# gooey-audio/libgooey

Hardware: NVIDIA B200
Metric: voice-samples/sec (higher is better)
Workload: dtype f32

## Files before the change

libgooey_b200/csrc/kernels.cuh:

```cuda
#pragma once
#include <cuda_runtime.h>
#include "voices2.cuh"
#include "../../include/gooey_batch.h"

namespace gd {

constexpr int TILE = 32;

template <class S> __device__ __forceinline__ void load_words(S& s, const uint32_t* base, int slot, int n_pad, int w0) {
  constexpr int W = sizeof(S) / 4;
  uint32_t* w = reinterpret_cast<uint32_t*>(&s);
#pragma unroll
  for (int i = 0; i < W; i++) w[i] = base[(size_t)(w0 + i) * n_pad + slot];
}
template <class S> __device__ __forceinline__ void store_words(const S& s, uint32_t* base, int slot, int n_pad, int w0) {
  constexpr int W = sizeof(S) / 4;
  const uint32_t* w = reinterpret_cast<const uint32_t*>(&s);
#pragma unroll
  for (int i = 0; i < W; i++) base[(size_t)(w0 + i) * n_pad + slot] = w[i];
}

struct KickV {
  using State = KickState; using Ctl = KickCtl; using Aud = KickAud; using Span = KickSpan;
  static constexpr bool FAST = true; static constexpr int NPL = KICK_PLANES; static constexpr uint32_t ID = GOOEY_INSTRUMENT_KICK;
  struct Run { KickDer d; int j_act; };
  static __device__ __forceinline__ float tick(State& s, const double* tt, const RateCtx& rc) { return kick_tick(s, tt, rc); }
  static __device__ __forceinline__ void slow_event(State& s, const VoiceEvent& e, const double* tt, const RateCtx&) {
    uint32_t r = 0; kick_event(s.c, e, tt, r); kick_span_begin(s.a, s.c, r);
  }
  static __device__ __forceinline__ bool settled(const Ctl& c) { return params_settled<K_NP>(c.cur, c.tgt); }
  static __device__ __forceinline__ void event(Ctl& c, const VoiceEvent& e, const double* tt, uint32_t& r) { kick_event(c, e, tt, r); }
  static __device__ __forceinline__ void plan(Ctl& c, uint32_t r, const double* tt, int ja, int jb, Span& sp) { kick_plan(c, r, tt, ja, jb, sp); }
  static __device__ __forceinline__ int front_end(const Span& sp) { return sp.j_act; }
  static __device__ __forceinline__ void front(const Span& sp, double now, uint32_t, float sr, float* o) {
// ... 108 lines not shown
  const VoiceEvent* events;
  const uint32_t* ev_begin;
  const double* tt;
  int frames;
  float* out; long long stride;
  RateCtx rc;
  uint8_t* mode;
  void* spans;
  const uint32_t* span_off;
  uint32_t* n_spans;
  uint32_t* span_cursor;
  float* planes;
  long long plane_stride;
  int pitch;
  int chunk0, chunk_frames;
  const ModRoute* routes; const uint32_t* route_begin;
  const float* mod_planes; long long mod_pitch; int mod_frame0;
};

__device__ __forceinline__ void store_tile_voice_major(const float* tile , float* out, long long stride, int row0,
                                                        const uint32_t* rows, uint32_t row_mask, int f0, int nf, int lane) {
  const bool vec_ok = (nf == TILE) && ((stride & 3) == 0) && ((f0 & 3) == 0) && ((reinterpret_cast<uintptr_t>(out) & 15) == 0);
  if (vec_ok) {
    const int c = (lane & 7) * 4;
#pragma unroll
    for (int k = 0; k < 8; k++) {
      const int r = k * 4 + (lane >> 3);
      if ((row_mask >> r) & 1u) {
        const float* src = tile + r * 33 + c;
        float4 v = make_float4(src[0], src[1], src[2], src[3]);
// ... 6 lines not shown
      if (!((row_mask >> r) & 1u)) continue;
      const long long row = rows ? (long long)rows[r] : (long long)(row0 + r);
      if (lane < nf) out[row * stride + f0 + lane] = tile[r * 33 + lane];
    }
  }
}
__device__ __forceinline__ void load_tile_rows(float* tile , const float* plane, int pitch, int row0, int n_rows, int c0, int lane) {
  const int c = (lane & 7) * 4;
#pragma unroll
  for (int k = 0; k < 8; k++) {
    const int r = k * 4 + (lane >> 3);
    if (r < n_rows) {
      const float4 v = *reinterpret_cast<const float4*>(plane + (size_t)(row0 + r) * pitch + c0 + c);
      float* dst = tile + r * 33 + c;
      dst[0] = v.x; dst[1] = v.y; dst[2] = v.z; dst[3] = v.w;
    }
  }
}

__device__ __forceinline__ void load_tile_rows_any(float* tile , const float* plane, long long pitch, int row0, int n_rows, int c0, int nf, int lane) {
  for (int r = 0; r < n_rows; r++)
    if (lane < nf) tile[r * 33 + lane] = plane[(long long)(row0 + r) * pitch + c0 + lane];
}

template <class V, int BLOCK>
__global__ void __launch_bounds__(BLOCK) slow_kernel(const VoiceLaunch L) {
  __shared__ float tiles[BLOCK / 32][TILE * 33];
  const int v = blockIdx.x * BLOCK + threadIdx.x;
  const int lane = threadIdx.x & 31;
  const int warp = threadIdx.x >> 5;
// ... 177 lines not shown
```

libgooey_b200/csrc/pool.cuh:

```cuda
#pragma once
#include <algorithm>
#include <atomic>
#include <map>
#include <type_traits>
#include <mutex>
#include <tuple>
#include "device_rt.h"
#include "wave.cuh"
#include "coop.cuh"
#include "gran_wave.cuh"
#include "bass_wave.cuh"
#include "poly_wave.cuh"
#include "patch.h"

namespace gh {

extern std::atomic<uint64_t> g_launches;

struct KernelStat { uint64_t launches = 0; double ms = 0.0; double voice_frames = 0.0; };
std::map<std::string, KernelStat>& kernel_stats();
std::mutex& kernel_stats_mutex();
struct KernelTimer {
  struct Rec { cudaEvent_t t0, t1; const char* key; double units; };
  std::vector<Rec> recs;
// ... 134 lines not shown
  }
};
ClockTable& clock_table(float sr);

enum class Back { Wave, Coop, Serial };
constexpr int COOP_FROM = 4096;
constexpr int COOP_NV = 16;
constexpr int SERIAL_FROM = 12288;
inline bool serial_backend() { const char* e = getenv("GOOEY_B200_BACKEND"); return e && strcmp(e, "serial") == 0; }
template <class V> inline Back choose_back(int cnt) {
  if (serial_backend()) return Back::Serial;
  if (std::is_same<V, gd::TomV>::value) return cnt >= COOP_FROM ? Back::Coop : Back::Wave;
  return cnt >= SERIAL_FROM ? Back::Serial : Back::Wave;
}
template <class V> struct WaveOf;
template <> struct WaveOf<gd::KickV> { using W = gd::wave::KickW; static constexpr const char* name = "wave_kernel<KickW>"; };
template <> struct WaveOf<gd::SnareV> { using W = gd::wave::SnareW; static constexpr const char* name = "wave_kernel<SnareW>"; };
template <> struct WaveOf<gd::HatV> { using W = gd::wave::HatW; static constexpr const char* name = "wave_kernel<HatW>"; };
template <> struct WaveOf<gd::TomV> { using W = gd::wave::TomW; static constexpr const char* name = "wave_kernel<TomW>"; };

inline void coop_launch(int cnt, cudaStream_t s, const gd::VoiceLaunch& L) {
  using SM = gd::coop::Smem<gd::coop::TomC, COOP_NV>;
  auto kernel = gd::coop::coop_kernel<gd::coop::TomC, COOP_NV>;
  func_attr_once((const void*)kernel, cudaFuncAttributeMaxDynamicSharedMemorySize, (int)sizeof(SM));
  func_attr_once((const void*)kernel, cudaFuncAttributePreferredSharedMemoryCarveout, (int)cudaSharedmemCarveoutMaxShared);
  kernel<<<(cnt + COOP_NV - 1) / COOP_NV, COOP_NV * 32, sizeof(SM), s>>>(L);
}

template <class K> inline void same_carveout(K kernel) {
  func_attr_once((const void*)kernel, cudaFuncAttributePreferredSharedMemoryCarveout, (int)cudaSharedmemCarveoutMaxShared);
}
#define GH_LAUNCH(kernel, grid, block, stream, ...) do { same_carveout(kernel); kernel<<<grid, block, 0, stream>>>(__VA_ARGS__); } while (0)

template <class V> inline void slow_launch(const gd::VoiceLaunch& L, cudaStream_t s) {
// ... 23 lines not shown
template <> inline const char* launch_back<gd::GranV>(const gd::VoiceLaunch& L, cudaStream_t s) {
  GH_LAUNCH((gd::gran_wave_kernel<4>), (L.n + 3) / 4, 128, s, L);
  return "gran_wave_kernel";
}

constexpr int CHUNK_FRAMES = 8192;
template <class V> struct TypeRunner {
  using State = typename V::State;
  Pool<State> pool;
  std::vector<uint32_t> slots, rows, ev_begin, span_off;
  std::vector<gd::VoiceEvent> ev_flat;
  std::vector<gd::ModRoute> routes_flat; std::vector<uint32_t> route_begin;
  DevBuf<gd::ModRoute> d_routes; DevBuf<uint32_t> d_route_begin;
  const float* mod_planes = nullptr; long long mod_pitch = 0; int mod_frame0 = 0;
  DevBuf<uint32_t> d_slots, d_rows, d_ev_begin, d_span_off, d_n_spans, d_span_cursor;
  DevBuf<gd::VoiceEvent> d_events;
  DevBuf<uint8_t> d_mode, d_spans;
  DevBuf<float> d_planes[2];
  cudaStream_t sB = nullptr, sC = nullptr, sS = nullptr;
  cudaEvent_t evA = nullptr, evB[2] = {nullptr, nullptr}, evC[2] = {nullptr, nullptr}, evDoneC = nullptr, evDoneS = nullptr;
  KernelTimer timer;
  std::vector<cudaEvent_t> evChunk;
  int launched_chunks = 0;
  static int chunk_of(int frames) { return std::min(CHUNK_FRAMES, (frames + 31) & ~31); }
  void wait_chunk(cudaStream_t s, int i) {
    if (n() == 0) return;
    if (launched_chunks == 0) { GH_CUDA(cudaStreamWaitEvent(s, evDoneC, 0)); return; }
    GH_CUDA(cudaStreamWaitEvent(s, evDoneS, 0));
    GH_CUDA(cudaStreamWaitEvent(s, evChunk[std::min(i, launched_chunks - 1)], 0));
  }
// ... 46 lines not shown
    memset(&L, 0, sizeof L);
    L.state = pool.d.p; L.n = cnt; L.n_pad = pool.cap;
    L.slots = d_slots.p; L.rows = d_rows.p; L.row0 = 0;
    L.events = d_events.p; L.ev_begin = d_ev_begin.p; L.tt = tt; L.frames = frames; L.out = out; L.stride = stride; L.rc = rc;
    if (!routes_flat.empty() && mod_planes) {
      d_routes.upload(routes_flat.data(), routes_flat.size(), sC);
      d_route_begin.upload(route_begin.data(), route_begin.size(), sC);
      L.routes = d_routes.p; L.route_begin = d_route_begin.p; L.mod_planes = mod_planes; L.mod_pitch = mod_pitch; L.mod_frame0 = mod_frame0;
    }
    const char* key = nullptr;
    if constexpr (V::FAST) {
      using Span = typename V::Span;
      d_span_off.upload(span_off.data(), span_off.size(), sC);
      d_n_spans.alloc(cnt); d_span_cursor.alloc(cnt); d_mode.alloc(cnt);
      d_spans.alloc((size_t)span_off.back() * sizeof(Span));
      const int chunk = chunk_of(frames);
      const int rows_pad = pad32(cnt);
      const size_t plane_floats = (size_t)rows_pad * chunk;
      d_planes[0].alloc(plane_floats * V::NPL); d_planes[1].alloc(plane_floats * V::NPL);
      L.mode = d_mode.p; L.spans = d_spans.p; L.span_off = d_span_off.p; L.n_spans = d_n_spans.p; L.span_cursor = d_span_cursor.p;
      L.plane_stride = (long long)plane_floats; L.pitch = chunk;
      GH_LAUNCH((gd::plan_kernel<V>), (cnt + 63) / 64, 64, sC, L);
      g_launches.fetch_add(1, std::memory_order_relaxed);
      GH_CUDA(cudaGetLastError());
      GH_CUDA(cudaEventRecord(evA, sC));
      GH_CUDA(cudaStreamWaitEvent(sB, evA, 0));
      GH_CUDA(cudaStreamWaitEvent(sS, evA, 0));
      GH_LAUNCH((gd::slow_kernel<V, 32>), (cnt + 31) / 32, 32, sS, L);
      g_launches.fetch_add(1, std::memory_order_relaxed);
      GH_CUDA(cudaGetLastError());
      GH_CUDA(cudaEventRecord(evDoneS, sS));
      int i = 0;
      for (int c0 = 0; c0 < frames; c0 += chunk, i++) {
        const int b = i & 1;
        L.chunk0 = c0; L.chunk_frames = std::min(chunk, frames - c0);
        L.planes = d_planes[b].p;
        if (i >= 2) GH_CUDA(cudaStreamWaitEvent(sB, evC[b], 0));
        const int bpv = (L.chunk_frames + 255) / 256;
        GH_LAUNCH((gd::front_kernel<V, 256>), (unsigned)((size_t)cnt * bpv), 256, sB, L, bpv);
        GH_CUDA(cudaGetLastError());
        GH_CUDA(cudaEventRecord(evB[b], sB));
        GH_CUDA(cudaStreamWaitEvent(sC, evB[b], 0));
        timer.begin(sC);
        key = launch_back<V>(L, sC);
        GH_CUDA(cudaGetLastError());
        timer.end(sC, key, (double)cnt * L.chunk_frames);
        GH_CUDA(cudaEventRecord(evC[b], sC));
        if ((int)evChunk.size() <= i) { cudaEvent_t e; GH_CUDA(cudaEventCreateWithFlags(&e, cudaEventDisableTiming)); evChunk.push_back(e); }
        GH_CUDA(cudaEventRecord(evChunk[i], sC));
        g_launches.fetch_add(2, std::memory_order_relaxed);
      }
      launched_chunks = i;
    } else {
      timer.begin(sC);
      key = launch_back<V>(L, sC);
// ... 50 lines not shown
```

libgooey_b200/csrc/voices.cuh:

```cuda
#pragma once
#include "dsp.cuh"
#include "events.h"

namespace gd {

struct RateCtx {
  float sr;
  double dt;
  float smooth15;
  float smooth10, smooth30, smooth50;
  float click_alpha;
  float asym_down;
  PinkCoef pink;
};
G_HD RateCtx make_rate_ctx(float sr) {
  RateCtx c;
  c.sr = sr;
  c.dt = 1.0 / (double)sr;
  c.smooth15 = smooth_coeff(sr, 15.0f);
  c.smooth10 = smooth_coeff(sr, 10.0f);
  c.smooth30 = smooth_coeff(sr, 30.0f);
  c.smooth50 = smooth_coeff(sr, 50.0f);
  c.click_alpha = 1.0f - gm::g_expf(-2.0f * PI_F * 8000.0f / sr);
  c.asym_down = 1.0f - gm::g_expf(-1.0f / 100.0f);
// ... 195 lines not shown
  a.click_hp += rc.click_alpha * hp;
  float filt_click = hp * (1.0f + 4.0f * 0.1f);
  float noise_out = 0.0f;
  if (d.noise_amount > 0.001f) {
    float pn = pink_tick(a.pink, rc.pink);
    rlp_set(a.noise_lp, sr, d.noise_cut, d.noise_res);
    float fn = rlp_process(a.noise_lp, pn);
    noise_out = fn * f.ne * d.noise_amount * 0.5f;
  }
  float total = f.p1 + filt_click + noise_out;
  a.ws.drive = d.drive;
  a.ws.feedback = d.feedback;
  fbws_set_cutoff(a.ws, sr, d.fb_cutoff);
  float od = fbws_process(a.ws, total);
  return od * f.amp * d.va * d.volume;
}
G_D float kick_tick(KickState& s, const double* tt, const RateCtx& rc) {
  KickCtl& c = s.c;
  const double now = tt[c.k];
  c.k += 1;
#pragma unroll
  for (int i = 0; i < K_NP; i++) smooth_tick(c.cur[i], c.tgt[i], rc.smooth15);
  if (!c.active) return 0.0f;
  kick_live(c);
  const KickDer d = kick_derive(c);
#ifdef __CUDA_ARCH__
  const KickFront f = d.drive <= 8.0f ? kick_front<true>(c, d, now, rc.sr) : kick_front<false>(c, d, now, rc.sr);
#else
  const KickFront f = kick_front(c, d, now, rc.sr);
#endif
// ... 191 lines not shown
}
G_HD bool snare_still_active(const SnareCtl& c) {
  bool classic = env_active(c.tonal_osc_env) || env_active(c.noise_osc_env) || env_active(c.crack_env);
  bool ds = env_active(c.tonal_env) || env_active(c.main_noise_env) || env_active(c.tail_env) || env_active(c.amp_env) || c.pm.active;
  return classic || ds;
}
G_D float snare_back(SnareAud& a, const SnareDer& d, const SnareFront& f, const RateCtx& rc) {
  chamb_set(a.filt, rc.sr, d.cutoff, d.res);
  float filtered = chamb_process(a.filt, f.raw_noise, d.filter_type);
  float noise_out = filtered * f.cne * d.noise_mix;
  float total = f.tonal_out + noise_out + f.crack_out;
  a.ws.drive = d.drive;
  float od = ws_process(a.ws, total);
  return od * f.amp * d.va * d.volume;
}
G_D float snare_tick(SnareState& s, const double* tt, const RateCtx& rc) {
  SnareCtl& c = s.c;
  const double now = tt[c.k];
  c.k += 1;
  bool changing = false;
#pragma unroll
  for (int i = 0; i < S_NP; i++) { smooth_tick(c.cur[i], c.tgt[i], rc.smooth15); changing |= (c.cur[i] != c.tgt[i]); }
  if (!c.active) return 0.0f;
  if (changing) {
    float cvs = 0.7f + 0.3f * c.velocity;
    c.tonal_vol = clampf(c.cur[S_TONAL], 0.0f, 1.0f);
    c.noise_vol = clampf(c.cur[S_NOISE] * 0.8f, 0.0f, 1.0f);
    c.crack_vol = clampf(c.cur[S_BRIGHTNESS] * 0.4f * cvs, 0.0f, 1.0f);
  }
  snare_live(c);
// ... 135 lines not shown
  else { float n = u64_to_f32(xorshift64s_next(a.white)) / 18446744073709551616.0f; noise = (n * 2.0f) - 1.0f; }
  float mod_out = hat_osc(a.mod_phase, d.pitch_hz * 0.1f, sr, noise * 0.25f);
  float main_out = hat_osc(a.main_phase, d.pitch_hz, sr, mod_out * 0.75f);
  hp_set(a.hp1, sr, d.pitch_hz, 1.0f);
  float filtered = biquad_process(a.hp1, main_out);
  if (d.db24) { hp_set(a.hp2, sr, d.pitch_hz, 1.0f); filtered = biquad_process(a.hp2, filtered) * 0.8f; }
  float env = f.env;
  if (env >= a.env_smooth) a.env_smooth = env; else a.env_smooth += rc.asym_down * (env - a.env_smooth);
  env = a.env_smooth;
  float out = filtered * env * d.vel035 * 0.35f;
  tpt_set(a.svf, sr, d.tone_hz, 0.5f);
  float lo, bd, hi;
  tpt_process(a.svf, out, lo, bd, hi);
  float o = hi * d.volume;
  if (env_complete && a.env_smooth < 1e-4f) a.active = 0;
  return o;
}
G_D float hat_tick(HatState& s, const double* tt, const RateCtx& rc) {
  HatCtl& c = s.c;
  const double now = tt[c.k];
  c.k += 1;
#pragma unroll
  for (int i = 0; i < H_NP; i++) smooth_tick(c.cur[i], c.tgt[i], rc.smooth15);
  if (!s.a.active) return 0.0f;
  hat_live(c);
  const HatDer d = hat_derive(c);
  HatFront f;
  f.env = maxenv_value(c.env, now);
  return hat_back(s.a, d, f, maxenv_complete(c.env), rc);
}
// ... 273 lines not shown
```

libgooey_b200/csrc/wave.cuh:

```cuda
#pragma once
#include "kernels.cuh"

namespace gd { namespace wave {

__device__ __forceinline__ float shup(float v, int d) { return __shfl_up_sync(0xffffffffu, v, d); }
__device__ __forceinline__ float shl(float v, int n) { return __shfl_sync(0xffffffffu, v, n); }
__device__ __forceinline__ bool gall(bool p) { return __all_sync(0xffffffffu, p); }
__device__ __forceinline__ unsigned gballot(bool p) { return __ballot_sync(0xffffffffu, p); }
__device__ __forceinline__ void gsync() { __syncwarp(); }

struct Geo1 { float m[5]; float ap; };
struct Geo2 { float a; float m[5]; float ap; };

__device__ __forceinline__ Geo1 make_geo1(float a, int lane) {
  Geo1 g; float p = a, ap = 1.0f; const int e = lane + 1;
#pragma unroll
  for (int i = 0; i < 5; i++) { g.m[i] = lane >= (1 << i) ? p : 0.0f; if (e & (1 << i)) ap *= p; p *= p; }
  if (e & 32) ap *= p;
  g.ap = ap;
  return g;
}
__device__ __forceinline__ Geo2 make_geo2(float a, int lane) {
  Geo2 g; g.a = a; float p = a * a, ap = 1.0f;
#pragma unroll
// ... 147 lines not shown

__device__ __forceinline__ float w_tanh(float x) {
  const float ax = fabsf(x);
  const float e = __expf(2.0f * ax);
  const float t = 1.0f - __fdividef(2.0f, e + 1.0f);
  return copysignf(t, x);
}
__device__ __forceinline__ float w_gain_comp(FbShaper& w, float env) {
  const float reference = fmaxf(env, 0.05f);
  const float driven = fmaxf(fabsf(w_tanh(reference * w.drive)), 1e-6f);
  const float comp_no_fb = w_tanh(reference) / driven;
  const float makeup = fbws_makeup(w);
  const float taming = 1.0f / (1.0f + comp_no_fb * w.feedback * 0.25f);
  return fminf(comp_no_fb * taming * makeup, 3.0f);
}
__device__ __forceinline__ float wrap01(float x) { return x < 1.0f ? x : (x < 2.0f ? x - 1.0f : fmodf(x, 1.0f)); }

struct TptLin { float in0, in1; };
__device__ __forceinline__ TptLin tpt_lin_init(Lin2& S, const Tpt& f, int lane) {
  const float g = f.g, h = f.h, gh = g * h, g2h = g * gh;
  lin2_init(S, 2.0f * h - 1.0f, -2.0f * gh, 2.0f * gh, 1.0f - 2.0f * g2h, lane);
  TptLin t; t.in0 = 2.0f * gh; t.in1 = 2.0f * g2h;
  return t;
}
__device__ __forceinline__ void tpt_scan(const Lin2& S, const TptLin& t, Tpt& f, float in, float& ic1_pre, float& ic2_pre, int lane, int last) {
  float s0 = t.in0 * in, s1 = t.in1 * in;
  lin2_scan(S, s0, s1, f.ic1, f.ic2, lane);
  ic1_pre = prev_lane(s0, f.ic1, lane); ic2_pre = prev_lane(s1, f.ic2, lane);
  f.ic1 = shl(s0, last); f.ic2 = shl(s1, last);
}
__device__ __forceinline__ void biquad_lin_init(Lin2& S, const Biquad& b, int lane) { lin2_init(S, -b.a1, -b.a2, 1.0f, 0.0f, lane); }
// ... 3 lines not shown
  xm2 = lane == 0 ? b.x2 : (lane == 1 ? b.x1 : xm2);
  float f0 = b.b0 * x + b.b1 * xm1 + b.b2 * xm2, f1 = 0.0f;
  lin2_scan(S, f0, f1, b.y1, b.y2, lane);
  const float nx1 = shl(x, last), nx2 = shl(xm1, last);
  const float ny1 = shl(f0, last), ny2 = shl(f1, last);
  b.x1 = nx1; b.x2 = nx2; b.y1 = ny1; b.y2 = ny2;
  return fabsf(f0) < 1e-15f ? 0.0f : f0;
}

#define LANE_VAL(v, n) shl((v), (n))
#define STASH_PUT(slot, v) (sc.stash[slot][lane] = (v))
#define STASH_GET(slot, n) (sc.stash[slot][n])

struct KickW {
  using V = KickV;
  struct Span2 { bool noise, shaper, serial; };
  static __device__ __forceinline__ int active_end(const KickV::Run& r) { return r.j_act; }
  static __device__ __forceinline__ void span_setup(KickAud& a, const KickV::Run& r, Span2& w, WaveScratch&, const RateCtx& rc, int) {
    w.noise = r.d.noise_amount > 0.001f;
    a.ws.drive = r.d.drive; a.ws.feedback = r.d.feedback;
    fbws_set_cutoff(a.ws, rc.sr, r.d.fb_cutoff);
    w.shaper = !(a.ws.mix <= 0.0001f || a.ws.drive <= 1.0f);
    w.serial = w.shaper && a.ws.feedback != 0.0f;
    if (w.noise) rlp_set(a.noise_lp, rc.sr, r.d.noise_cut, r.d.noise_res);
  }
  static __device__ __forceinline__ float block(KickAud& a, const KickV::Run& r, const Span2& w, WaveScratch& sc, const GeoTables& T,
                                                const float* p, int, int& nl, const RateCtx& rc, int lane) {
    const int last = nl - 1;
    const float p1 = p[0], raw_click = p[1], ne = p[2], amp = p[3];
    float hp_l = 0.0f, fn_l = 0.0f;
    gsync(); STASH_PUT(0, raw_click); gsync();
#pragma unroll 4
    for (int n = 0; n < nl; n++) {
      const float raw = STASH_GET(0, n);
      const float hp = raw - a.click_hp;
      a.click_hp += rc.click_alpha * hp;
      float fn = 0.0f;
      if (w.noise) fn = rlp_process(a.noise_lp, pink_tick(a.pink, rc.pink));
      if (n == lane) { hp_l = hp; fn_l = fn; }
    }
    const float filt_click = hp_l * (1.0f + 4.0f * 0.1f);
    const float noise_out = w.noise ? fn_l * ne * r.d.noise_amount * 0.5f : 0.0f;
    const float total = p1 + filt_click + noise_out;
    float od = total;
    const bool finite = gall(isfinite(total));
    if (w.serial || (w.shaper && !finite)) {
#pragma unroll 4
      for (int n = 0; n < nl; n++) {
        const float y = fbws_process(a.ws, LANE_VAL(total, n));
        if (n == lane) od = y;
      }
    } else if (w.shaper) {
      FbShaper& ws = a.ws;
      const float fb_in = ws.drive * total + ws.feedback * ws.last_out;
      const float shaped = os_scan(ws.os, fb_in, [](float x) { return w_tanh(x); }, T, lane, last);
      const float rect_l = fabsf(total);
      float env_l = 0.0f;
// ... 17 lines not shown
        ws.dc_x1 = c;
        ws.dc_y1 = fabsf(out) < 1e-15f ? 0.0f : out;
        ws.filter_state += ws.filter_coeff * (out - ws.filter_state);
        if (fabsf(ws.filter_state) < 1e-15f) ws.filter_state = 0.0f;
        if (n == lane) out_l = out;
      }
      ws.last_out = ws.filter_state;
      od = total * (1.0f - ws.mix) + out_l * ws.mix;
    }
    return od * amp * r.d.va * r.d.volume;
  }
};

struct SnareW {
  using V = SnareV;
  struct Span2 { float comp; bool shaper; };
  static __device__ __forceinline__ int active_end(const SnareV::Run& r) { return r.j_act; }
  static __device__ __forceinline__ void span_setup(SnareAud& a, const SnareV::Run& r, Span2& w, WaveScratch&, const RateCtx& rc, int) {
    chamb_set(a.filt, rc.sr, r.d.cutoff, r.d.res);
    a.ws.drive = r.d.drive;
    w.shaper = !(a.ws.mix <= 0.0001f || a.ws.drive <= 1.0f);
    w.comp = w.shaper ? gm::g_tanhf(0.5f) / gm::g_tanhf(0.5f * a.ws.drive) : 1.0f;
  }
  static __device__ __forceinline__ float block(SnareAud& a, const SnareV::Run& r, const Span2& w, WaveScratch& sc, const GeoTables& T,
                                                const float* p, int, int& nl, const RateCtx&, int lane) {
    const int last = nl - 1;
    const float tonal_out = p[0], raw_noise = p[1], cne = p[2], crack_out = p[3], amp = p[4];
    float low_l = 0.0f, band_l = 0.0f, high_l = 0.0f;
    {
      const float f = a.filt.f, q = a.filt.q;
      float low = a.filt.low, band = a.filt.band;
      gsync(); STASH_PUT(0, raw_noise); gsync();
#pragma unroll 4
      for (int n = 0; n < nl; n++) {
        const float in = STASH_GET(0, n);
        float high = 0.0f;
#pragma unroll
        for (int i = 0; i < 2; i++) { low = low + f * band; high = in - low - q * band; band = f * high + band; }
        if (n == lane) { low_l = low; band_l = band; high_l = high; }
      }
      a.filt.low = low; a.filt.band = band;
    }
    const float filtered = svf_pick(low_l, band_l, high_l, r.d.filter_type);
    const float noise_out = filtered * cne * r.d.noise_mix;
    const float total = tonal_out + noise_out + crack_out;
    float od = total;
    const bool finite = gall(isfinite(total));
    if (!finite) {
#pragma unroll 4
      for (int n = 0; n < nl; n++) {
        const float y = ws_process(a.ws, LANE_VAL(total, n));
        if (n == lane) od = y;
      }
    } else if (w.shaper) {
      const float d = a.ws.drive, comp = w.comp;
      const float sat = os_scan(a.ws.os, total, [d, comp](float x) { return w_tanh(x * d) * comp; }, T, lane, last);
      od = total * (1.0f - a.ws.mix) + sat * a.ws.mix;
    }
    return od * amp * r.d.va * r.d.volume;
  }
};

struct HatW {
  using V = HatV;
  struct Span2 { TptLin svf; };
  static __device__ __forceinline__ int active_end(const HatV::Run&) { return 0x7fffffff; }
  static __device__ __forceinline__ void span_setup(HatAud& a, const HatV::Run& r, Span2& w, WaveScratch& sc, const RateCtx& rc, int lane) {
    hp_set(a.hp1, rc.sr, r.d.pitch_hz, 1.0f);
    biquad_lin_init(sc.lin[0], a.hp1, lane);
    if (r.d.db24) { hp_set(a.hp2, rc.sr, r.d.pitch_hz, 1.0f); biquad_lin_init(sc.lin[1], a.hp2, lane); }
    tpt_set(a.svf, rc.sr, r.d.tone_hz, 0.5f);
    w.svf = tpt_lin_init(sc.lin[2], a.svf, lane);
  }
  static __device__ __forceinline__ float block(HatAud& a, const HatV::Run& r, const Span2& w, WaveScratch& sc, const GeoTables&,
                                                const float* p, int j, int& nl, const RateCtx& rc, int lane) {
    const float sr = rc.sr;
    const float env_l = (j + lane) < r.j_env ? p[0] : r.env_final;
    float es_l = 0.0f;
    int nv = nl;
    gsync(); STASH_PUT(0, env_l); gsync();
    if (j + nl <= r.j_env) {
#pragma unroll 4
      for (int n = 0; n < nl; n++) {
        const float e = STASH_GET(0, n);
        if (e >= a.env_smooth) a.env_smooth = e; else a.env_smooth += rc.asym_down * (e - a.env_smooth);
        if (n == lane) es_l = a.env_smooth;
      }
    } else {
#pragma unroll 4
      for (int n = 0; n < nl; n++) {
        const float e = STASH_GET(0, n);
        if (e >= a.env_smooth) a.env_smooth = e; else a.env_smooth += rc.asym_down * (e - a.env_smooth);
        if (n == lane) es_l = a.env_smooth;
        if ((j + n) >= r.j_env && a.env_smooth < 1e-4f) { nv = n + 1; a.active = 0; break; }
      }
    }
    nl = nv;
    float noise = 0.0f, mph = 0.0f, nph = 0.0f;
    const float inc_mod = fmaxf(r.d.pitch_hz * 0.1f, 0.0f) / sr, inc_main = fmaxf(r.d.pitch_hz, 0.0f) / sr;
    const bool small_inc = inc_main < 1.0f && a.mod_phase < 1.0f && a.main_phase < 1.0f;
    if (!r.d.pink_on && small_inc) {
      uint64_t st_l = 0;
#pragma unroll 4
      for (int n = 0; n < nv; n++) {
        uint64_t x = a.white;
        x ^= x >> 12; x ^= x << 25; x ^= x >> 27;
        a.white = x;
        float pm = a.mod_phase + inc_mod; a.mod_phase = pm < 1.0f ? pm : pm - 1.0f;
        float pn = a.main_phase + inc_main; a.main_phase = pn < 1.0f ? pn : pn - 1.0f;
        if (n == lane) { st_l = x; mph = a.mod_phase; nph = a.main_phase; }
      }
      const float u = u64_to_f32(st_l * 0x2545f4914f6cdd1dull) / 18446744073709551616.0f;
      noise = (u * 2.0f) - 1.0f;
    } else {
#pragma unroll 4
      for (int n = 0; n < nv; n++) {
        float x;
        if (r.d.pink_on) x = pink_tick(a.pink, rc.pink);
        else { float u = u64_to_f32(xorshift64s_next(a.white)) / 18446744073709551616.0f; x = (u * 2.0f) - 1.0f; }
        a.mod_phase = wrap01(a.mod_phase + inc_mod);
        a.main_phase = wrap01(a.main_phase + inc_main);
        if (n == lane) { noise = x; mph = a.mod_phase; nph = a.main_phase; }
      }
    }
    float ph = mph + noise * 0.25f; ph -= floorf(ph);
    const float mod_out = gm::g_sinf(2.0f * PI_F * ph);
    ph = nph + mod_out * 0.75f; ph -= floorf(ph);
    const float main_out = gm::g_sinf(2.0f * PI_F * ph);
    const int last = nv - 1;
    float filtered = biquad_scan(sc.lin[0], a.hp1, main_out, lane, last);
    if (r.d.db24) filtered = biquad_scan(sc.lin[1], a.hp2, filtered, lane, last) * 0.8f;
    const float out = filtered * es_l * r.d.vel035 * 0.35f;
    float ic1p, ic2p;
    tpt_scan(sc.lin[2], w.svf, a.svf, out, ic1p, ic2p, lane, last);
    const float v1 = (a.svf.g * (out - ic2p) + ic1p) * a.svf.h;
    const float v2 = ic2p + a.svf.g * v1;
    const float hi = out - (a.svf.r * v1 + v2);
    return hi * r.d.volume;
  }
};

struct TomW {
  using V = TomV;
  struct Span2 { int dummy; };
  static __device__ __forceinline__ int active_end(const TomV::Run&) { return 0x7fffffff; }
  static __device__ __forceinline__ void span_setup(TomAud&, const TomV::Run&, Span2&, WaveScratch&, const RateCtx&, int) {}
  static __device__ __forceinline__ float generic(TomAud& a, const TomV::Run& r, WaveScratch& sc, float env_l, float noise_l, float rnd_l,
                                                  int j, int& nl, const RateCtx& rc, int lane) {
    float y_l = 0.0f;
    int nv = nl;
    gsync(); STASH_PUT(0, env_l); STASH_PUT(1, noise_l); STASH_PUT(2, rnd_l); gsync();
#pragma unroll 2
    for (int n = 0; n < nl; n++) {
      TomFront f; f.env = STASH_GET(0, n); f.noise = STASH_GET(1, n); f.rnd = STASH_GET(2, n);
      const float y = tom_back(a, r.d, f, (j + n) >= r.j_env, rc);
      if (n == lane) y_l = y;
      if (!a.active) { nv = n + 1; break; }
    }
    nl = nv;
    return y_l;
// ... 170 lines not shown

template <class W>
__global__ void __launch_bounds__(32, 1) wave_kernel(const VoiceLaunch L) {
  using V = typename W::V; using Span = typename V::Span; using Aud = typename V::Aud;
  constexpr int WC = sizeof(typename V::Ctl) / 4;
  __shared__ GeoTables T;
  __shared__ WaveScratch sc;
  const int lane = threadIdx.x & 31;
  geo_tables_init(T, L.rc, threadIdx.x, 32);
  __syncthreads();
  const int v = blockIdx.x;
  const bool alive = v < L.n && L.mode[v] == 0;
  const int sv = alive ? (L.slots ? (int)L.slots[v] : v) : 0;
  Aud a;
  const Span* spans = nullptr;
  uint32_t ns = 0, cur = 0xffffffffu;
  typename V::Run run;
  typename W::Span2 w2;
  bool ready = false;
  int next_j0 = 0x7fffffff;
  float* out = nullptr;
  const float* planes = nullptr;
  if (alive) {
    load_words(a, L.state, sv, L.n_pad, WC);
    spans = reinterpret_cast<const Span*>(L.spans) + L.span_off[v];
    ns = L.n_spans[v];
    cur = L.span_cursor[v];
    if (cur != 0xffffffffu) V::span_resume(spans[cur], run);
    next_j0 = cur + 1u < ns ? spans[cur + 1u].j0 : 0x7fffffff;
    const long long row = L.rows ? (long long)L.rows[v] : (long long)(L.row0 + v);
    out = L.out + row * L.stride;
    planes = L.planes + (size_t)v * L.pitch;
  }
  const int c1 = L.chunk0 + min(L.chunk_frames, L.frames - L.chunk0);
  int j = L.chunk0;
  while (alive && j < c1) {
    while (j == next_j0) {
      cur += 1u;
      V::span_begin(a, spans[cur], run, L.rc.sr);
      ready = false;
      next_j0 = cur + 1u < ns ? spans[cur + 1u].j0 : 0x7fffffff;
    }
    const int span_end = min(next_j0, c1);
    const int act_end = min(span_end, W::active_end(run));
    if (cur == 0xffffffffu || !V::is_active(a, run, j) || j >= act_end) {
      for (int k = j + lane; k < span_end; k += 32) out[k] = 0.0f;
      j = span_end;
      continue;
    }
    if (!ready) { gsync(); W::span_setup(a, run, w2, sc, L.rc, lane); ready = true; }
    int nl = min(32, act_end - j);
    float p[V::NPL];
    const int jj = j + min(lane, nl - 1);
#pragma unroll
    for (int q = 0; q < V::NPL; q++) p[q] = planes[(size_t)q * L.plane_stride + (jj - L.chunk0)];
    const float y = W::block(a, run, w2, sc, T, p, j, nl, L.rc, lane);
    if (lane < nl) out[j + lane] = y;
    j += nl;
  }
  if (alive && lane == 0) {
    store_words(a, L.state, sv, L.n_pad, WC);
    L.span_cursor[v] = cur;
  }
}

#undef LANE_VAL
} }
```

Baseline: 8.873 billion.

## Split serial per-voice recurrences into a thread-per-voice replay kernel before wave kernel

Adds a replay kernel that runs the cheap serial recurrences (kick click HP and pink noise LP, snare chamberlin filter, hat envelope smoothing, noise and phase accumulators) with one thread per voice. Results are rewritten into the front planes. The warp-per-voice wave kernel then reads these precomputed values instead of running the serial loops on lane 0 with shuffles/stash. State words are split so each kernel loads and stores only its part, and hat activity cut points are recorded per span. This removes serial work from the wave kernel, at the cost of an extra launch and extra plane traffic.

```diff
diff --git a/libgooey_b200/csrc/kernels.cuh b/libgooey_b200/csrc/kernels.cuh
--- a/libgooey_b200/csrc/kernels.cuh
+++ b/libgooey_b200/csrc/kernels.cuh
@@ -7,17 +7,17 @@
 
 constexpr int TILE = 32;
 
-template <class S> __device__ __forceinline__ void load_words(S& s, const uint32_t* base, int slot, int n_pad, int w0) {
-  constexpr int W = sizeof(S) / 4;
+template <class S, int LO = 0, int HI = (int)(sizeof(S) / 4)>
+__device__ __forceinline__ void load_words(S& s, const uint32_t* base, int slot, int n_pad, int w0) {
   uint32_t* w = reinterpret_cast<uint32_t*>(&s);
 #pragma unroll
-  for (int i = 0; i < W; i++) w[i] = base[(size_t)(w0 + i) * n_pad + slot];
-}
-template <class S> __device__ __forceinline__ void store_words(const S& s, uint32_t* base, int slot, int n_pad, int w0) {
-  constexpr int W = sizeof(S) / 4;
+  for (int i = LO; i < HI; i++) w[i] = base[(size_t)(w0 + i) * n_pad + slot];
+}
+template <class S, int LO = 0, int HI = (int)(sizeof(S) / 4)>
+__device__ __forceinline__ void store_words(const S& s, uint32_t* base, int slot, int n_pad, int w0) {
   const uint32_t* w = reinterpret_cast<const uint32_t*>(&s);
 #pragma unroll
-  for (int i = 0; i < W; i++) base[(size_t)(w0 + i) * n_pad + slot] = w[i];
+  for (int i = LO; i < HI; i++) base[(size_t)(w0 + i) * n_pad + slot] = w[i];
 }
 
 struct KickV {
@@ -156,6 +156,7 @@
   long long plane_stride;
   int pitch;
   int chunk0, chunk_frames;
+  int* span_cut;
   const ModRoute* routes; const uint32_t* route_begin;
   const float* mod_planes; long long mod_pitch; int mod_frame0;
 };
@@ -192,6 +193,18 @@
       const float4 v = *reinterpret_cast<const float4*>(plane + (size_t)(row0 + r) * pitch + c0 + c);
       float* dst = tile + r * 33 + c;
       dst[0] = v.x; dst[1] = v.y; dst[2] = v.z; dst[3] = v.w;
+    }
+  }
+}
+
+__device__ __forceinline__ void store_tile_rows(const float* tile , float* plane, int pitch, int row0, uint32_t row_mask, int c0, int lane) {
+  const int c = (lane & 7) * 4;
+#pragma unroll
+  for (int k = 0; k < 8; k++) {
+    const int r = k * 4 + (lane >> 3);
+    if ((row_mask >> r) & 1u) {
+      const float* src = tile + r * 33 + c;
+      *reinterpret_cast<float4*>(plane + (size_t)(row0 + r) * pitch + c0 + c) = make_float4(src[0], src[1], src[2], src[3]);
     }
   }
 }
diff --git a/libgooey_b200/csrc/pool.cuh b/libgooey_b200/csrc/pool.cuh
--- a/libgooey_b200/csrc/pool.cuh
+++ b/libgooey_b200/csrc/pool.cuh
@@ -172,10 +172,10 @@
   return cnt >= SERIAL_FROM ? Back::Serial : Back::Wave;
 }
 template <class V> struct WaveOf;
-template <> struct WaveOf<gd::KickV> { using W = gd::wave::KickW; static constexpr const char* name = "wave_kernel<KickW>"; };
-template <> struct WaveOf<gd::SnareV> { using W = gd::wave::SnareW; static constexpr const char* name = "wave_kernel<SnareW>"; };
-template <> struct WaveOf<gd::HatV> { using W = gd::wave::HatW; static constexpr const char* name = "wave_kernel<HatW>"; };
-template <> struct WaveOf<gd::TomV> { using W = gd::wave::TomW; static constexpr const char* name = "wave_kernel<TomW>"; };
+template <> struct WaveOf<gd::KickV> { using W = gd::wave::KickW; using R = gd::KickR; static constexpr const char* name = "wave_kernel<KickW>"; };
+template <> struct WaveOf<gd::SnareV> { using W = gd::wave::SnareW; using R = gd::SnareR; static constexpr const char* name = "wave_kernel<SnareW>"; };
+template <> struct WaveOf<gd::HatV> { using W = gd::wave::HatW; using R = gd::HatR; static constexpr const char* name = "wave_kernel<HatW>"; };
+template <> struct WaveOf<gd::TomV> { using W = gd::wave::TomW; using R = void; static constexpr const char* name = "wave_kernel<TomW>"; };
 
 inline void coop_launch(int cnt, cudaStream_t s, const gd::VoiceLaunch& L) {
   using SM = gd::coop::Smem<gd::coop::TomC, COOP_NV>;
@@ -229,6 +229,7 @@
   DevBuf<gd::ModRoute> d_routes; DevBuf<uint32_t> d_route_begin;
   const float* mod_planes = nullptr; long long mod_pitch = 0; int mod_frame0 = 0;
   DevBuf<uint32_t> d_slots, d_rows, d_ev_begin, d_span_off, d_n_spans, d_span_cursor;
+  DevBuf<int> d_span_cut;
   DevBuf<gd::VoiceEvent> d_events;
   DevBuf<uint8_t> d_mode, d_spans;
   DevBuf<float> d_planes[2];
@@ -305,12 +306,19 @@
       d_span_off.upload(span_off.data(), span_off.size(), sC);
       d_n_spans.alloc(cnt); d_span_cursor.alloc(cnt); d_mode.alloc(cnt);
       d_spans.alloc((size_t)span_off.back() * sizeof(Span));
+      using R = typename WaveOf<V>::R;
+      constexpr bool has_replay = !std::is_void<R>::value;
+      const bool replay = has_replay && choose_back<V>(cnt) == Back::Wave;
       const int chunk = chunk_of(frames);
       const int rows_pad = pad32(cnt);
       const size_t plane_floats = (size_t)rows_pad * chunk;
-      d_planes[0].alloc(plane_floats * V::NPL); d_planes[1].alloc(plane_floats * V::NPL);
+      const int npl = std::max(V::NPL, WaveOf<V>::W::NPL);
+      d_planes[0].alloc(plane_floats * npl); d_planes[1].alloc(plane_floats * npl);
       L.mode = d_mode.p; L.spans = d_spans.p; L.span_off = d_span_off.p; L.n_spans = d_n_spans.p; L.span_cursor = d_span_cursor.p;
       L.plane_stride = (long long)plane_floats; L.pitch = chunk;
+      if constexpr (has_replay) {
+        if (replay && R::CUTS) { d_span_cut.alloc(span_off.back()); L.span_cut = d_span_cut.p; }
+      }
       GH_LAUNCH((gd::plan_kernel<V>), (cnt + 63) / 64, 64, sC, L);
       g_launches.fetch_add(1, std::memory_order_relaxed);
       GH_CUDA(cudaGetLastError());
@@ -330,6 +338,13 @@
         const int bpv = (L.chunk_frames + 255) / 256;
         GH_LAUNCH((gd::front_kernel<V, 256>), (unsigned)((size_t)cnt * bpv), 256, sB, L, bpv);
         GH_CUDA(cudaGetLastError());
+        if constexpr (has_replay) {
+          if (replay) {
+            GH_LAUNCH((gd::replay_kernel<R>), (cnt + 31) / 32, 32, sB, L);
+            GH_CUDA(cudaGetLastError());
+            g_launches.fetch_add(1, std::memory_order_relaxed);
+          }
+        }
         GH_CUDA(cudaEventRecord(evB[b], sB));
         GH_CUDA(cudaStreamWaitEvent(sC, evB[b], 0));
         timer.begin(sC);
diff --git a/libgooey_b200/csrc/replay.cuh b/libgooey_b200/csrc/replay.cuh
--- /dev/null
+++ b/libgooey_b200/csrc/replay.cuh
@@ -0,0 +1,117 @@
+#pragma once
+#include <cstddef>
+#include "kernels.cuh"
+
+namespace gd {
+
+struct KickR {
+  using V = KickV;
+  static constexpr int P0 = 1, NIN = 2, NOUT = 2;
+  static constexpr int LO = 0, HI = offsetof(KickAud, ws) / 4, LO2 = 0, HI2 = 0;
+  static constexpr bool CUTS = false;
+  static __device__ __forceinline__ bool active(const KickAud&, const KickV::Run& r, int j) { return j < r.j_act; }
+  static __device__ __forceinline__ void begin(const KickAud&, int, int*) {}
+  static __device__ __forceinline__ void frame(KickAud& a, const KickV::Run& r, int, float* x, int*, const RateCtx& rc) {
+    float filt_click, noise_out;
+    kick_replay(a, r.d, x[0], x[1], rc, filt_click, noise_out);
+    x[0] = filt_click; x[1] = noise_out;
+  }
+};
+struct SnareR {
+  using V = SnareV;
+  static constexpr int P0 = 1, NIN = 1, NOUT = 1;
+  static constexpr int LO = 0, HI = offsetof(SnareAud, ws) / 4, LO2 = 0, HI2 = 0;
+  static constexpr bool CUTS = false;
+  static __device__ __forceinline__ bool active(const SnareAud&, const SnareV::Run& r, int j) { return j < r.j_act; }
+  static __device__ __forceinline__ void begin(const SnareAud&, int, int*) {}
+  static __device__ __forceinline__ void frame(SnareAud& a, const SnareV::Run& r, int, float* x, int*, const RateCtx& rc) {
+    x[0] = snare_replay(a, r.d, x[0], rc);
+  }
+};
+struct HatR {
+  using V = HatV;
+  static constexpr int P0 = 0, NIN = 1, NOUT = 4;
+  static constexpr int LO = 0, HI = offsetof(HatAud, hp1) / 4;
+  static constexpr int LO2 = offsetof(HatAud, white) / 4, HI2 = sizeof(HatAud) / 4;
+  static constexpr bool CUTS = true;
+  static __device__ __forceinline__ bool active(const HatAud& a, const HatV::Run&, int) { return a.active != 0; }
+  static __device__ __forceinline__ void begin(const HatAud& a, int j, int* cut) { *cut = a.active ? 0x7fffffff : j; }
+  static __device__ __forceinline__ void frame(HatAud& a, const HatV::Run& r, int j, float* x, int* cut, const RateCtx& rc) {
+    const HatRep o = hat_replay(a, r.d, j < r.j_env ? x[0] : r.env_final, j >= r.j_env, rc);
+    x[0] = o.env; x[1] = o.noise; x[2] = o.mod_phase; x[3] = o.main_phase;
+    if (!a.active) *cut = j + 1;
+  }
+};
+
+template <class R>
+__global__ void __launch_bounds__(32) replay_kernel(const VoiceLaunch L) {
+  using V = typename R::V; using Span = typename V::Span; using Aud = typename V::Aud;
+  constexpr int WC = sizeof(typename V::Ctl) / 4;
+  static_assert(R::NIN <= R::NOUT, "planes are rewritten in place");
+  __shared__ float tiles[R::NOUT][TILE * 33];
+  const int lane = threadIdx.x;
+  const int v0 = blockIdx.x * 32, v = v0 + lane;
+  const bool mine = v < L.n && L.mode[v] == 0;
+  if (__ballot_sync(0xffffffffu, mine) == 0u) return;
+  const int n_rows = min(32, L.n - v0);
+  Aud a;
+  typename V::Run run;
+  const Span* spans = nullptr;
+  uint32_t cur = 0xffffffffu, ns = 0;
+  int next_j0 = 0x7fffffff, sv = v;
+  int* cuts = nullptr;
+  if (mine) {
+    if (L.slots) sv = (int)L.slots[v];
+    load_words<Aud, R::LO, R::HI>(a, L.state, sv, L.n_pad, WC);
+    load_words<Aud, R::LO2, R::HI2>(a, L.state, sv, L.n_pad, WC);
+    spans = reinterpret_cast<const Span*>(L.spans) + L.span_off[v];
+    ns = L.n_spans[v];
+    if (R::CUTS) cuts = L.span_cut + L.span_off[v];
+    if (L.chunk0 > 0) {
+      int lo = 0, hi = (int)ns - 1;
+      while (lo < hi) { const int mid = (lo + hi + 1) >> 1; if (spans[mid].j0 < L.chunk0) lo = mid; else hi = mid - 1; }
+      cur = (uint32_t)lo;
+      V::span_resume(spans[cur], run);
+    }
+    next_j0 = cur + 1u < ns ? spans[cur + 1u].j0 : 0x7fffffff;
+  }
+  const int cend = min(L.chunk_frames, L.frames - L.chunk0);
+  for (int f0 = 0; f0 < cend; f0 += TILE) {
+    const int nf = min(TILE, cend - f0);
+    const int j0 = L.chunk0 + f0;
+    const bool want = mine && ((cur != 0xffffffffu && R::active(a, run, j0)) || next_j0 < j0 + nf);
+    const uint32_t want_mask = __ballot_sync(0xffffffffu, want);
+    if (want_mask == 0u) continue;
+#pragma unroll
+    for (int p = 0; p < R::NIN; p++) load_tile_rows(tiles[p], L.planes + (size_t)(R::P0 + p) * L.plane_stride, L.pitch, v0, n_rows, f0, lane);
+    __syncwarp();
+    if (want) {
+      for (int jj = 0; jj < nf; jj++) {
+        const int j = j0 + jj;
+        while (j == next_j0) {
+          cur += 1u;
+          V::span_begin(a, spans[cur], run, L.rc.sr);
+          R::begin(a, j, cuts + cur);
+          next_j0 = cur + 1u < ns ? spans[cur + 1u].j0 : 0x7fffffff;
+        }
+        if (!R::active(a, run, j)) continue;
+        float x[R::NOUT];
+#pragma unroll
+        for (int q = 0; q < R::NIN; q++) x[q] = tiles[q][lane * 33 + jj];
+        R::frame(a, run, j, x, cuts + cur, L.rc);
+#pragma unroll
+        for (int q = 0; q < R::NOUT; q++) tiles[q][lane * 33 + jj] = x[q];
+      }
+    }
+    __syncwarp();
+#pragma unroll
+    for (int p = 0; p < R::NOUT; p++) store_tile_rows(tiles[p], L.planes + (size_t)(R::P0 + p) * L.plane_stride, L.pitch, v0, want_mask, f0, lane);
+    __syncwarp();
+  }
+  if (mine) {
+    store_words<Aud, R::LO, R::HI>(a, L.state, sv, L.n_pad, WC);
+    store_words<Aud, R::LO2, R::HI2>(a, L.state, sv, L.n_pad, WC);
+  }
+}
+
+}
diff --git a/libgooey_b200/csrc/voices.cuh b/libgooey_b200/csrc/voices.cuh
--- a/libgooey_b200/csrc/voices.cuh
+++ b/libgooey_b200/csrc/voices.cuh
@@ -233,6 +233,18 @@
   fbws_set_cutoff(a.ws, sr, d.fb_cutoff);
   float od = fbws_process(a.ws, total);
   return od * f.amp * d.va * d.volume;
+}
+G_D void kick_replay(KickAud& a, const KickDer& d, float raw_click, float ne, const RateCtx& rc, float& filt_click, float& noise_out) {
+  float hp = raw_click - a.click_hp;
+  a.click_hp += rc.click_alpha * hp;
+  filt_click = hp * (1.0f + 4.0f * 0.1f);
+  noise_out = 0.0f;
+  if (d.noise_amount > 0.001f) {
+    float pn = pink_tick(a.pink, rc.pink);
+    rlp_set(a.noise_lp, rc.sr, d.noise_cut, d.noise_res);
+    float fn = rlp_process(a.noise_lp, pn);
+    noise_out = fn * ne * d.noise_amount * 0.5f;
+  }
 }
 G_D float kick_tick(KickState& s, const double* tt, const RateCtx& rc) {
   KickCtl& c = s.c;
@@ -454,6 +466,10 @@
   float od = ws_process(a.ws, total);
   return od * f.amp * d.va * d.volume;
 }
+G_D float snare_replay(SnareAud& a, const SnareDer& d, float raw_noise, const RateCtx& rc) {
+  chamb_set(a.filt, rc.sr, d.cutoff, d.res);
+  return chamb_process(a.filt, raw_noise, d.filter_type);
+}
 G_D float snare_tick(SnareState& s, const double* tt, const RateCtx& rc) {
   SnareCtl& c = s.c;
   const double now = tt[c.k];
@@ -619,6 +635,19 @@
   tpt_process(a.svf, out, lo, bd, hi);
   float o = hi * d.volume;
   if (env_complete && a.env_smooth < 1e-4f) a.active = 0;
+  return o;
+}
+G_HD float wrap01(float x) { return x < 1.0f ? x : (x < 2.0f ? x - 1.0f : fmodf(x, 1.0f)); }
+struct HatRep { float env, noise, mod_phase, main_phase; };
+G_D HatRep hat_replay(HatAud& a, const HatDer& d, float env, bool env_complete, const RateCtx& rc) {
+  HatRep o;
+  if (d.pink_on) o.noise = pink_tick(a.pink, rc.pink);
+  else { float n = u64_to_f32(xorshift64s_next(a.white)) / 18446744073709551616.0f; o.noise = (n * 2.0f) - 1.0f; }
+  a.mod_phase = wrap01(a.mod_phase + fmaxf(d.pitch_hz * 0.1f, 0.0f) / rc.sr);
+  a.main_phase = wrap01(a.main_phase + fmaxf(d.pitch_hz, 0.0f) / rc.sr);
+  if (env >= a.env_smooth) a.env_smooth = env; else a.env_smooth += rc.asym_down * (env - a.env_smooth);
+  if (env_complete && a.env_smooth < 1e-4f) a.active = 0;
+  o.env = a.env_smooth; o.mod_phase = a.mod_phase; o.main_phase = a.main_phase;
   return o;
 }
 G_D float hat_tick(HatState& s, const double* tt, const RateCtx& rc) {
diff --git a/libgooey_b200/csrc/wave.cuh b/libgooey_b200/csrc/wave.cuh
--- a/libgooey_b200/csrc/wave.cuh
+++ b/libgooey_b200/csrc/wave.cuh
@@ -1,5 +1,6 @@
 #pragma once
-#include "kernels.cuh"
+#include <cstddef>
+#include "replay.cuh"
 
 namespace gd { namespace wave {
 
@@ -185,7 +186,6 @@
   const float taming = 1.0f / (1.0f + comp_no_fb * w.feedback * 0.25f);
   return fminf(comp_no_fb * taming * makeup, 3.0f);
 }
-__device__ __forceinline__ float wrap01(float x) { return x < 1.0f ? x : (x < 2.0f ? x - 1.0f : fmodf(x, 1.0f)); }
 
 struct TptLin { float in0, in1; };
 __device__ __forceinline__ TptLin tpt_lin_init(Lin2& S, const Tpt& f, int lane) {
@@ -219,33 +219,20 @@
 
 struct KickW {
   using V = KickV;
-  struct Span2 { bool noise, shaper, serial; };
-  static __device__ __forceinline__ int active_end(const KickV::Run& r) { return r.j_act; }
+  static constexpr int NPL = KICK_PLANES;
+  static constexpr int LO = offsetof(KickAud, ws) / 4, HI = sizeof(KickAud) / 4;
+  struct Span2 { bool shaper, serial; };
+  static __device__ __forceinline__ int active_end(const KickAud&, const KickV::Run& r, int) { return r.j_act; }
   static __device__ __forceinline__ void span_setup(KickAud& a, const KickV::Run& r, Span2& w, WaveScratch&, const RateCtx& rc, int) {
-    w.noise = r.d.noise_amount > 0.001f;
     a.ws.drive = r.d.drive; a.ws.feedback = r.d.feedback;
     fbws_set_cutoff(a.ws, rc.sr, r.d.fb_cutoff);
     w.shaper = !(a.ws.mix <= 0.0001f || a.ws.drive <= 1.0f);
     w.serial = w.shaper && a.ws.feedback != 0.0f;
-    if (w.noise) rlp_set(a.noise_lp, rc.sr, r.d.noise_cut, r.d.noise_res);
   }
   static __device__ __forceinline__ float block(KickAud& a, const KickV::Run& r, const Span2& w, WaveScratch& sc, const GeoTables& T,
-                                                const float* p, int, int& nl, const RateCtx& rc, int lane) {
+                                                const float* p, int, int& nl, const RateCtx&, int lane) {
     const int last = nl - 1;
-    const float p1 = p[0], raw_click = p[1], ne = p[2], amp = p[3];
-    float hp_l = 0.0f, fn_l = 0.0f;
-    gsync(); STASH_PUT(0, raw_click); gsync();
-#pragma unroll 4
-    for (int n = 0; n < nl; n++) {
-      const float raw = STASH_GET(0, n);
-      const float hp = raw - a.click_hp;
-      a.click_hp += rc.click_alpha * hp;
-      float fn = 0.0f;
-      if (w.noise) fn = rlp_process(a.noise_lp, pink_tick(a.pink, rc.pink));
-      if (n == lane) { hp_l = hp; fn_l = fn; }
-    }
-    const float filt_click = hp_l * (1.0f + 4.0f * 0.1f);
-    const float noise_out = w.noise ? fn_l * ne * r.d.noise_amount * 0.5f : 0.0f;
+    const float p1 = p[0], filt_click = p[1], noise_out = p[2], amp = p[3];
     const float total = p1 + filt_click + noise_out;
     float od = total;
     const bool finite = gall(isfinite(total));
@@ -293,10 +280,11 @@
 
 struct SnareW {
   using V = SnareV;
+  static constexpr int NPL = SNARE_PLANES;
+  static constexpr int LO = offsetof(SnareAud, ws) / 4, HI = sizeof(SnareAud) / 4;
   struct Span2 { float comp; bool shaper; };
-  static __device__ __forceinline__ int active_end(const SnareV::Run& r) { return r.j_act; }
-  static __device__ __forceinline__ void span_setup(SnareAud& a, const SnareV::Run& r, Span2& w, WaveScratch&, const RateCtx& rc, int) {
-    chamb_set(a.filt, rc.sr, r.d.cutoff, r.d.res);
+  static __device__ __forceinline__ int active_end(const SnareAud&, const SnareV::Run& r, int) { return r.j_act; }
+  static __device__ __forceinline__ void span_setup(SnareAud& a, const SnareV::Run& r, Span2& w, WaveScratch&, const RateCtx&, int) {
     a.ws.drive = r.d.drive;
     w.shaper = !(a.ws.mix <= 0.0001f || a.ws.drive <= 1.0f);
     w.comp = w.shaper ? gm::g_tanhf(0.5f) / gm::g_tanhf(0.5f * a.ws.drive) : 1.0f;
@@ -304,23 +292,7 @@
   static __device__ __forceinline__ float block(SnareAud& a, const SnareV::Run& r, const Span2& w, WaveScratch& sc, const GeoTables& T,
                                                 const float* p, int, int& nl, const RateCtx&, int lane) {
     const int last = nl - 1;
-    const float tonal_out = p[0], raw_noise = p[1], cne = p[2], crack_out = p[3], amp = p[4];
-    float low_l = 0.0f, band_l = 0.0f, high_l = 0.0f;
-    {
-      const float f = a.filt.f, q = a.filt.q;
-      float low = a.filt.low, band = a.filt.band;
-      gsync(); STASH_PUT(0, raw_noise); gsync();
-#pragma unroll 4
-      for (int n = 0; n < nl; n++) {
-        const float in = STASH_GET(0, n);
-        float high = 0.0f;
-#pragma unroll
-        for (int i = 0; i < 2; i++) { low = low + f * band; high = in - low - q * band; band = f * high + band; }
-        if (n == lane) { low_l = low; band_l = band; high_l = high; }
-      }
-      a.filt.low = low; a.filt.band = band;
-    }
-    const float filtered = svf_pick(low_l, band_l, high_l, r.d.filter_type);
+    const float tonal_out = p[0], filtered = p[1], cne = p[2], crack_out = p[3], amp = p[4];
     const float noise_out = filtered * cne * r.d.noise_mix;
     const float total = tonal_out + noise_out + crack_out;
     float od = total;
@@ -342,8 +314,10 @@
 
 struct HatW {
   using V = HatV;
+  static constexpr int NPL = HatR::NOUT;
+  static constexpr int LO = offsetof(HatAud, hp1) / 4, HI = offsetof(HatAud, white) / 4;
   struct Span2 { TptLin svf; };
-  static __device__ __forceinline__ int active_end(const HatV::Run&) { return 0x7fffffff; }
+  static __device__ __forceinline__ int active_end(const HatAud&, const HatV::Run&, int cut) { return cut; }
   static __device__ __forceinline__ void span_setup(HatAud& a, const HatV::Run& r, Span2& w, WaveScratch& sc, const RateCtx& rc, int lane) {
     hp_set(a.hp1, rc.sr, r.d.pitch_hz, 1.0f);
     biquad_lin_init(sc.lin[0], a.hp1, lane);
@@ -352,61 +326,13 @@
     w.svf = tpt_lin_init(sc.lin[2], a.svf, lane);
   }
   static __device__ __forceinline__ float block(HatAud& a, const HatV::Run& r, const Span2& w, WaveScratch& sc, const GeoTables&,
-                                                const float* p, int j, int& nl, const RateCtx& rc, int lane) {
-    const float sr = rc.sr;
-    const float env_l = (j + lane) < r.j_env ? p[0] : r.env_final;
-    float es_l = 0.0f;
-    int nv = nl;
-    gsync(); STASH_PUT(0, env_l); gsync();
-    if (j + nl <= r.j_env) {
-#pragma unroll 4
-      for (int n = 0; n < nl; n++) {
-        const float e = STASH_GET(0, n);
-        if (e >= a.env_smooth) a.env_smooth = e; else a.env_smooth += rc.asym_down * (e - a.env_smooth);
-        if (n == lane) es_l = a.env_smooth;
-      }
-    } else {
-#pragma unroll 4
-      for (int n = 0; n < nl; n++) {
-        const float e = STASH_GET(0, n);
-        if (e >= a.env_smooth) a.env_smooth = e; else a.env_smooth += rc.asym_down * (e - a.env_smooth);
-        if (n == lane) es_l = a.env_smooth;
-        if ((j + n) >= r.j_env && a.env_smooth < 1e-4f) { nv = n + 1; a.active = 0; break; }
-      }
-    }
-    nl = nv;
-    float noise = 0.0f, mph = 0.0f, nph = 0.0f;
-    const float inc_mod = fmaxf(r.d.pitch_hz * 0.1f, 0.0f) / sr, inc_main = fmaxf(r.d.pitch_hz, 0.0f) / sr;
-    const bool small_inc = inc_main < 1.0f && a.mod_phase < 1.0f && a.main_phase < 1.0f;
-    if (!r.d.pink_on && small_inc) {
-      uint64_t st_l = 0;
-#pragma unroll 4
-      for (int n = 0; n < nv; n++) {
-        uint64_t x = a.white;
-        x ^= x >> 12; x ^= x << 25; x ^= x >> 27;
-        a.white = x;
-        float pm = a.mod_phase + inc_mod; a.mod_phase = pm < 1.0f ? pm : pm - 1.0f;
-        float pn = a.main_phase + inc_main; a.main_phase = pn < 1.0f ? pn : pn - 1.0f;
-        if (n == lane) { st_l = x; mph = a.mod_phase; nph = a.main_phase; }
-      }
-      const float u = u64_to_f32(st_l * 0x2545f4914f6cdd1dull) / 18446744073709551616.0f;
-      noise = (u * 2.0f) - 1.0f;
-    } else {
-#pragma unroll 4
-      for (int n = 0; n < nv; n++) {
-        float x;
-        if (r.d.pink_on) x = pink_tick(a.pink, rc.pink);
-        else { float u = u64_to_f32(xorshift64s_next(a.white)) / 18446744073709551616.0f; x = (u * 2.0f) - 1.0f; }
-        a.mod_phase = wrap01(a.mod_phase + inc_mod);
-        a.main_phase = wrap01(a.main_phase + inc_main);
-        if (n == lane) { noise = x; mph = a.mod_phase; nph = a.main_phase; }
-      }
-    }
+                                                const float* p, int, int& nl, const RateCtx&, int lane) {
+    const float es_l = p[0], noise = p[1], mph = p[2], nph = p[3];
     float ph = mph + noise * 0.25f; ph -= floorf(ph);
     const float mod_out = gm::g_sinf(2.0f * PI_F * ph);
     ph = nph + mod_out * 0.75f; ph -= floorf(ph);
     const float main_out = gm::g_sinf(2.0f * PI_F * ph);
-    const int last = nv - 1;
+    const int last = nl - 1;
     float filtered = biquad_scan(sc.lin[0], a.hp1, main_out, lane, last);
     if (r.d.db24) filtered = biquad_scan(sc.lin[1], a.hp2, filtered, lane, last) * 0.8f;
     const float out = filtered * es_l * r.d.vel035 * 0.35f;
@@ -422,7 +348,9 @@
 struct TomW {
   using V = TomV;
   struct Span2 { int dummy; };
-  static __device__ __forceinline__ int active_end(const TomV::Run&) { return 0x7fffffff; }
+  static constexpr int NPL = TOM_PLANES;
+  static constexpr int LO = 0, HI = sizeof(TomAud) / 4;
+  static __device__ __forceinline__ int active_end(const TomAud& a, const TomV::Run&, int) { return a.active ? 0x7fffffff : -1; }
   static __device__ __forceinline__ void span_setup(TomAud&, const TomV::Run&, Span2&, WaveScratch&, const RateCtx&, int) {}
   static __device__ __forceinline__ float generic(TomAud& a, const TomV::Run& r, WaveScratch& sc, float env_l, float noise_l, float rnd_l,
                                                   int j, int& nl, const RateCtx& rc, int lane) {
@@ -623,7 +551,9 @@
   const int sv = alive ? (L.slots ? (int)L.slots[v] : v) : 0;
   Aud a;
   const Span* spans = nullptr;
+  const int* cuts = nullptr;
   uint32_t ns = 0, cur = 0xffffffffu;
+  int cut = 0x7fffffff;
   typename V::Run run;
   typename W::Span2 w2;
   bool ready = false;
@@ -631,11 +561,12 @@
   float* out = nullptr;
   const float* planes = nullptr;
   if (alive) {
-    load_words(a, L.state, sv, L.n_pad, WC);
+    load_words<Aud, W::LO, W::HI>(a, L.state, sv, L.n_pad, WC);
     spans = reinterpret_cast<const Span*>(L.spans) + L.span_off[v];
+    if (L.span_cut) cuts = L.span_cut + L.span_off[v];
     ns = L.n_spans[v];
     cur = L.span_cursor[v];
-    if (cur != 0xffffffffu) V::span_resume(spans[cur], run);
+    if (cur != 0xffffffffu) { V::span_resume(spans[cur], run); if (cuts) cut = cuts[cur]; }
     next_j0 = cur + 1u < ns ? spans[cur + 1u].j0 : 0x7fffffff;
     const long long row = L.rows ? (long long)L.rows[v] : (long long)(L.row0 + v);
     out = L.out + row * L.stride;
@@ -647,28 +578,29 @@
     while (j == next_j0) {
       cur += 1u;
       V::span_begin(a, spans[cur], run, L.rc.sr);
+      if (cuts) cut = cuts[cur];
       ready = false;
       next_j0 = cur + 1u < ns ? spans[cur + 1u].j0 : 0x7fffffff;
     }
     const int span_end = min(next_j0, c1);
-    const int act_end = min(span_end, W::active_end(run));
-    if (cur == 0xffffffffu || !V::is_active(a, run, j) || j >= act_end) {
+    const int act_end = min(span_end, W::active_end(a, run, cut));
+    if (cur == 0xffffffffu || j >= act_end) {
       for (int k = j + lane; k < span_end; k += 32) out[k] = 0.0f;
       j = span_end;
       continue;
     }
     if (!ready) { gsync(); W::span_setup(a, run, w2, sc, L.rc, lane); ready = true; }
     int nl = min(32, act_end - j);
-    float p[V::NPL];
+    float p[W::NPL];
     const int jj = j + min(lane, nl - 1);
 #pragma unroll
-    for (int q = 0; q < V::NPL; q++) p[q] = planes[(size_t)q * L.plane_stride + (jj - L.chunk0)];
+    for (int q = 0; q < W::NPL; q++) p[q] = planes[(size_t)q * L.plane_stride + (jj - L.chunk0)];
     const float y = W::block(a, run, w2, sc, T, p, j, nl, L.rc, lane);
     if (lane < nl) out[j + lane] = y;
     j += nl;
   }
   if (alive && lane == 0) {
-    store_words(a, L.state, sv, L.n_pad, WC);
+    store_words<Aud, W::LO, W::HI>(a, L.state, sv, L.n_pad, WC);
     L.span_cursor[v] = cur;
   }
 }
```

After: 5.636 billion, median of 6. 0.635x the previous value.
